# sxyu/pixel-nerf

Hardware: NVIDIA H100
Metric: rays/sec (64c+32f samples, 2 src views) (higher is better)
Workload: dtype f32 (fp16 hi/lo split products, fp32 accumulate)

## Files before the change

### pixel-nerf_b200/csrc/pnr_field_tc.cu

```cuda
#include <cuda_fp16.h>
#include <stdlib.h>

#include "pnr_common.cuh"
#include "pnr_geom.cuh"
#include "pnr_ray_ops.cuh"
#include "pnr_tc_ptx.cuh"

namespace pnr {

int sgemm(const float* A, int lda, const float* W, const float* bias, float* C, int ldc, int M, int N, int K,
          bool relu_a, bool accum, cudaStream_t s);
int gemm_f16x3(const float* A, int lda, const float* W, int ldw, const float* bias, float* C, int ldc, int M, int N, int K,
               cudaStream_t s);

namespace tc {

constexpr int D = 512;
constexpr int ROWS = 64;
constexpr int TILE_POINTS = 128;
constexpr int NCONSUMER_WARPS = 8;
constexpr int NCONSUMERS = NCONSUMER_WARPS * 32;
constexpr int NTHREADS = NCONSUMERS;
constexpr int SLOT_BYTES = 16384;
constexpr int HALF_SLOT_BYTES = SLOT_BYTES / 2;
constexpr int NSLOTS = 4;
constexpr int A_CHUNK_BYTES = 16384;
constexpr int A_BYTES = 8 * A_CHUNK_BYTES;
constexpr int AH_BYTES = 2 * A_CHUNK_BYTES;
constexpr int SLOTS_LIN_IN = 8;
constexpr int SLOTS_BLOCK = 128;
constexpr int SLOTS_TOTAL = SLOTS_LIN_IN + 5 * SLOTS_BLOCK;
constexpr int SLOTS_HEAD = SLOTS_LIN_IN + 3 * SLOTS_BLOCK;
constexpr int SLOTS_TAIL = 2 * SLOTS_BLOCK;
constexpr int HEADER_BYTES = 256;

constexpr int SM_A = 0;
constexpr int SM_AH = SM_A + A_BYTES;
constexpr int SM_B = SM_AH + AH_BYTES;
constexpr int SM_GEO = SM_B + NSLOTS * SLOT_BYTES;
constexpr int SM_PART = SM_A;
constexpr int SM_BAR = SM_GEO + ROWS * 8 * 4;
constexpr int BAR_FULL = 0;
constexpr int BAR_COUNT = BAR_FULL + NSLOTS;
constexpr int SM_NLIST = SM_BAR + 2 * BAR_COUNT * 8;
constexpr int SM_FEED = SM_NLIST + 16;
constexpr int FEED_BYTES = 128;
constexpr int SM_PROF = SM_FEED + 2 * FEED_BYTES;
#ifdef PNR_TC_PROFILE
constexpr int SMEM_BYTES = SM_PROF + 128;
#else
constexpr int SMEM_BYTES = SM_PROF;
#endif
static_assert(SMEM_BYTES <= 227 * 1024, "shared memory of one H100 block");
constexpr int FLUSH_SCRATCH_BYTES = A_BYTES / NCONSUMER_WARPS;


struct Pass {
  const uint8_t* packed;
  const float* proj;
  const float* fc0_b[5];
  const float* fc1_b[5];
  const float* lin_out_w;
  const float* lin_out_b;
  float* out;
  int64_t total_points;
  int64_t n_tiles;
  int64_t P;
  int K;
};

struct Render {
  const float* rays;
  const float *lin, *u_c, *u_f, *u_j, *n_d;
  float *zc, *wc, *zf;
  float *rgb_c, *depth_c, *rgb_f, *depth_f, *w_f;
  int* count;
  int* ready;
  int* lists;
  int64_t R;
  int cap, Kc, Kf, Kfd, white;
  float depth_std;
};

struct Params {
  PnrScene sc;
  PointSource src;
  Pass pass[2];
  Render rn;
  float* scratch;
  int npass;
  int* status;
};

using namespace tcptx;

enum { MODE_GATHER = 0, MODE_BIAS_WB = 1, MODE_COMBINE = 2, MODE_OUT = 3 };

#ifdef PNR_TC_PROFILE
extern __shared__ __align__(1024) uint8_t smem[];
enum { PH_FULL, PH_REFILL, PH_WGMMA_WAIT, PH_SYNC, PH_GATHER, PH_GEOM, PH_FLUSH, PH_TOTAL, PH_COUNT };
__device__ __forceinline__ void prof_add(int ph, long long t0, bool any_thread = false) {
  const long long dt = clock64() - t0;
  if (any_thread || (threadIdx.x & 127) == 0)
    reinterpret_cast<unsigned long long*>(smem + SM_PROF)[(threadIdx.x >> 7) * PH_COUNT + ph] += (unsigned long long)dt;
}
__device__ __forceinline__ void prof_finish(int* status, long long t_kernel) {
  prof_add(PH_TOTAL, t_kernel);
  if ((threadIdx.x & 127) == 0) {
    const unsigned long long* c = reinterpret_cast<const unsigned long long*>(smem + SM_PROF) + (threadIdx.x >> 7) * PH_COUNT;
    for (int i = 0; i < PH_COUNT; ++i) atomicAdd(reinterpret_cast<unsigned long long*>(status + 2) + i, c[i]);
  }
}
#define PROF_BEGIN(t) long long t = clock64()
#define PROF_RESTART(t) t = clock64()
#define PROF_END(ph, t) prof_add(ph, t)
#define PROF_END_ANY(ph, t) prof_add(ph, t, true)
#define PROF_INIT() \
  if (threadIdx.x < 2 * PH_COUNT) reinterpret_cast<unsigned long long*>(smem + SM_PROF)[threadIdx.x] = 0
#define PROF_FINISH(status, t) prof_finish(status, t)
#else
#define PROF_BEGIN(t)
#define PROF_RESTART(t)
#define PROF_END(ph, t)
#define PROF_END_ANY(ph, t)
#define PROF_INIT()
#define PROF_FINISH(status, t)
#endif

__device__ __forceinline__ void workers_sync() {
  PROF_BEGIN(t0);
  asm volatile("bar.sync 1, 256;" ::: "memory");
  PROF_END(PH_SYNC, t0);
}

__device__ __forceinline__ void st_evict_last(float* q, float v, uint64_t pol) {
  asm volatile("st.global.L2::cache_hint.f32 [%0], %1, %2;" ::"l"(q), "f"(v), "l"(pol) : "memory");
}
__device__ __forceinline__ float ld_evict_last(const float* q, uint64_t pol) {
  float v;
  asm volatile("ld.global.L2::cache_hint.f32 %0, [%1], %2;" : "=f"(v) : "l"(q), "l"(pol) : "memory");
  return v;
}
__device__ __forceinline__ float4 ldg_stream4(const float4* q, uint64_t pol) {
  float4 v;
  asm volatile("ld.global.nc.L2::cache_hint.v4.f32 {%0, %1, %2, %3}, [%4], %5;"
               : "=f"(v.x), "=f"(v.y), "=f"(v.z), "=f"(v.w)
               : "l"(q), "l"(pol));
  return v;
}
__device__ __forceinline__ void st_shared_u32(uint32_t saddr, uint32_t v) {
  asm volatile("st.shared.b32 [%0], %1;" ::"r"(saddr), "r"(v) : "memory");
}
__device__ __forceinline__ void split_relu2(float y0, float y1, uint32_t& hi, uint32_t& lo) {
  const float a0 = fmaxf(y0, 0.f), a1 = fmaxf(y1, 0.f);
  asm("cvt.rn.satfinite.f16x2.f32 %0, %1, %2;" : "=r"(hi) : "f"(a1), "f"(a0));
  const float2 hf = __half22float2(*reinterpret_cast<const __half2*>(&hi));
  asm("cvt.rn.satfinite.f16x2.f32 %0, %1, %2;" : "=r"(lo) : "f"(a1 - hf.y), "f"(a0 - hf.x));
}
__device__ __forceinline__ uint32_t relu_f16x2(float y0, float y1) {
  uint32_t hi;
  asm("cvt.rn.satfinite.f16x2.f32 %0, %1, %2;" : "=r"(hi) : "f"(fmaxf(y1, 0.f)), "f"(fmaxf(y0, 0.f)));
  return hi;
}
__device__ __forceinline__ uint32_t swz(int m, int k) {
  return (uint32_t)(m * 128 + ((((k >> 3) ^ (m & 7))) << 4) + (k & 7) * 2);
}

extern __shared__ __align__(1024) uint8_t smem[];

struct Feed {
  const uint8_t* src;
  uint64_t keep;
  int left;
  uint32_t released[2];
  const uint8_t* slots[2];
  int64_t n_tiles[2];
  int64_t tile;
  int npass, NS, pair, n_pairs;
  int ps, v;
  __device__ __forceinline__ void begin_run() {
    while (ps < npass && tile >= n_tiles[ps]) {
      ++ps;
      tile = pair;
    }
    const bool head = v < NS;
    src = ps < npass ? slots[ps] + (head ? 0 : (size_t)SLOTS_HEAD * SLOT_BYTES) : nullptr;
    left = (head ? SLOTS_HEAD : SLOTS_TAIL) / 2;
  }
  __device__ __forceinline__ void next_run() {
    if (++v > NS) {
      v = 0;
      tile += n_pairs;
    }
    begin_run();
  }
};
static_assert(sizeof(Feed) <= FEED_BYTES, "Feed does not fit its shared-memory slot");
static_assert(SLOTS_HEAD % 2 == 0 && SLOTS_TAIL % 2 == 0, "a step's two slots lie in one run");
static_assert(SM_PROF <= SMEM_BYTES, "the two rings' barriers and cursors fit under the block limit");
__device__ __forceinline__ Feed& feed(int wg) { return *reinterpret_cast<Feed*>(smem + SM_FEED + wg * FEED_BYTES); }

__device__ __forceinline__ uint32_t atom_add_acq_rel(uint32_t saddr, uint32_t v) {
  uint32_t old;
  asm volatile("atom.acq_rel.cta.shared::cta.add.u32 %0, [%1], %2;" : "=r"(old) : "r"(saddr), "r"(v) : "memory");
  return old;
}

template <bool FAST>
__device__ __forceinline__ void refill(uint32_t bar_base, uint32_t b_base, uint32_t n, int wg) {
  Feed& f = feed(wg);
  const uint8_t* src = f.src;
  if (src == nullptr) return;
  const uint64_t keep = f.keep;
  const uint32_t sl = n % NSLOTS;
#pragma unroll
  for (uint32_t k = 0; k < (FAST ? 1u : 2u); ++k) {
    const uint32_t full = bar_base + (BAR_FULL + sl + k) * 8;
    mbar_expect_tx(full, HALF_SLOT_BYTES);
    bulk_g2s_hint(b_base + (sl + k) * SLOT_BYTES, src + k * SLOT_BYTES, HALF_SLOT_BYTES, full, keep);
  }
  const int left = f.left - 1;
  f.left = left;
  if (left == 0)
    f.next_run();
  else
    f.src = src + 2 * SLOT_BYTES;
}

template <bool FAST>
struct Ring {
  uint32_t bar_base, b_base;
  uint32_t seq;
  uint32_t pend;
  bool has_pend;
  int lane;
  int* status;
  __device__ __forceinline__ uint32_t slot_addr(uint32_t s) const { return b_base + (s % NSLOTS) * SLOT_BYTES; }
  __device__ __forceinline__ void acquire() {
    if (has_pend) {
      PROF_BEGIN(t1);
      wgmma_wait<0>();
      PROF_END(PH_WGMMA_WAIT, t1);
      release(pend);
      has_pend = false;
    }
    PROF_BEGIN(t0);
    for (uint32_t s = seq; s < seq + (FAST ? 1 : 2); ++s)
      mbar_wait(bar_base + (BAR_FULL + s % NSLOTS) * 8, (s / NSLOTS) & 1, status,
                210 + 4 * (int)(threadIdx.x >> 7) + (int)(s % NSLOTS));
    PROF_END(PH_FULL, t0);
  }
  __device__ __forceinline__ void release(uint32_t s) {
    __syncwarp();
    if (lane == 0) {
      const int wg = threadIdx.x >> 7;
      if (atom_add_acq_rel(smem_u32(&feed(wg).released[(s / 2) & 1]), 1) % 4 == 3) {
        PROF_BEGIN(t0);
        refill<FAST>(bar_base, b_base, s + NSLOTS, wg);
        PROF_END_ANY(PH_REFILL, t0);
      }
    }
    __syncwarp();
  }
  __device__ __forceinline__ void issued() {
    wgmma_commit();
    pend = seq;
    has_pend = true;
    seq += 2;
  }
  __device__ __forceinline__ void drain() {
    PROF_BEGIN(t0);
    wgmma_wait<0>();
    PROF_END(PH_WGMMA_WAIT, t0);
    if (has_pend) release(pend);
    has_pend = false;
  }
};

template <bool FAST, int KSTEPS>
__device__ __forceinline__ void mma3(float* acc, uint64_t a_hi, uint64_t b_hi, uint64_t b_lo, bool zero) {
  const uint64_t a_lo = a_hi + (8192 >> 4);
#pragma unroll
  for (int kk = 0; kk < KSTEPS; ++kk) {
    wgmma_m64n64_f16(acc, a_hi + 2 * kk, b_hi + 2 * kk, (zero && kk == 0) ? 0u : 1u);
    if (FAST) continue;
    wgmma_m64n64_f16(acc, a_lo + 2 * kk, b_hi + 2 * kk, 1u);
    wgmma_m64n64_f16(acc, a_hi + 2 * kk, b_lo + 2 * kk, 1u);
  }
}

struct Cons {
  uint32_t smem_u;
  int tid, wg, lane;
  int r0, c0;
  float w_scale, w_inv;
  uint64_t l2_keep;
};

template <typename T>
__device__ __forceinline__ T* opaque(T* v) {
  asm volatile("" : "+l"(v));
  return v;
}
__device__ __forceinline__ uint32_t opaque(uint32_t v) {
  asm volatile("" : "+r"(v));
  return v;
}
__device__ __forceinline__ uint32_t acc_base(const Cons& c, uint32_t buf) {
  return opaque(c.smem_u + buf + c.wg * A_CHUNK_BYTES + swz(c.r0, c.c0));
}
__device__ __forceinline__ uint32_t acc_addr(uint32_t base, int q, int i) {
  return (base ^ (uint32_t)((i >> 2) << 4)) + q * 2 * A_CHUNK_BYTES + ((i >> 1) & 1) * 1024;
}

template <bool FAST, int KSTEPS>
__device__ __forceinline__ void wide_steps(Ring<FAST>& rg, const Cons& c, float (&x)[4][32], uint64_t a_hi,
                                           bool zero) {
  const uint64_t desc0 = make_desc(0);
#pragma unroll
  for (int q = 0; q < 4; ++q) {
    rg.acquire();
    const uint64_t b_hi = desc0 + (rg.slot_addr(rg.seq) >> 4);
    const uint64_t b_lo = desc0 + (rg.slot_addr(rg.seq + 1) >> 4);
    fence_acc<32>(x[q]);
    wgmma_fence();
    mma3<FAST, KSTEPS>(x[q], a_hi, b_hi, b_lo, zero);
    rg.issued();
  }
}

template <bool FAST>
__device__ __forceinline__ void fc_block(Ring<FAST>& rg, const Cons& c, float (&x)[4][32],
                                         const float* __restrict__ b0, const int* status) {
  const uint64_t desc0 = make_desc(0);
  float h[32];
#pragma unroll 1
  for (int hc = 0; hc < 4; ++hc) {
#pragma unroll 1
    for (int j = 0; j < 8; ++j) {
      rg.acquire();
      const uint64_t a_hi = desc0 + ((c.smem_u + SM_A + j * A_CHUNK_BYTES) >> 4);
      const uint64_t b_hi = desc0 + (rg.slot_addr(rg.seq) >> 4);
      const uint64_t b_lo = desc0 + (rg.slot_addr(rg.seq + 1) >> 4);
      fence_acc<32>(h);
      wgmma_fence();
      mma3<FAST, 4>(h, a_hi, b_hi, b_lo, j == 0);
      rg.issued();
    }
    rg.drain();
    fence_acc<32>(h);
    workers_sync();
    const float* bc = opaque(b0 + hc * 128 + c.wg * 64 + c.c0);
    const uint32_t ah = acc_base(c, SM_AH);
#pragma unroll
    for (int i = 0; i < 32; i += 2) {
      const float2 bb = __ldg(reinterpret_cast<const float2*>(bc + 8 * (i >> 2)));
      if (FAST) {
        st_shared_u32(acc_addr(ah, 0, i), relu_f16x2(h[i] * c.w_inv + bb.x, h[i + 1] * c.w_inv + bb.y));
        continue;
      }
      uint32_t hi, lo;
      split_relu2(h[i] * c.w_inv + bb.x, h[i + 1] * c.w_inv + bb.y, hi, lo);
      const uint32_t a = acc_addr(ah, 0, i);
      st_shared_u32(a, hi);
      st_shared_u32(a + 8192, lo);
    }
    fence_proxy_async();
    workers_sync();
#pragma unroll 1
    for (int jj = 0; jj < 2; ++jj)
      wide_steps<FAST, 4>(rg, c, x, desc0 + ((c.smem_u + SM_AH + jj * A_CHUNK_BYTES) >> 4), false);
  }
}

__device__ __forceinline__ void stage_gather(uint32_t smem_u, const float* __restrict__ proj_i, int warp, int lane) {
  const int sub = lane >> 4, l16 = lane & 15;
  uint64_t stream;
  asm volatile("createpolicy.fractional.L2::evict_first.b64 %0, 1.0;" : "=l"(stream));
#pragma unroll 1
  for (int j = 0; j < 8; ++j) {
    float4 t[4][4];
    uint32_t geo[4][4];
    float w[4][4];
#pragma unroll
    for (int it = 0; it < 4; ++it) {
      const uint32_t ga = smem_u + SM_GEO + (warp * 8 + it * 2 + sub) * 32;
#pragma unroll
      for (int k = 0; k < 4; ++k) {
        uint32_t wb;
        asm volatile("ld.shared.b32 %0, [%1];" : "=r"(geo[it][k]) : "r"(ga + 4 * k));
        asm volatile("ld.shared.b32 %0, [%1];" : "=r"(wb) : "r"(ga + 16 + 4 * k));
        w[it][k] = __uint_as_float(wb);
      }
    }
#pragma unroll
    for (int it = 0; it < 4; ++it)
#pragma unroll
      for (int k = 0; k < 4; ++k)
        t[it][k] = ldg_stream4(reinterpret_cast<const float4*>(proj_i + geo[it][k] + j * 64) + l16, stream);
#pragma unroll
    for (int it = 0; it < 4; ++it) {
      const int row = warp * 8 + it * 2 + sub;
      float4 g;
      g.x = ((t[it][0].x * w[it][0] + t[it][1].x * w[it][1]) + t[it][2].x * w[it][2]) + t[it][3].x * w[it][3];
      g.y = ((t[it][0].y * w[it][0] + t[it][1].y * w[it][1]) + t[it][2].y * w[it][2]) + t[it][3].y * w[it][3];
      g.z = ((t[it][0].z * w[it][0] + t[it][1].z * w[it][1]) + t[it][2].z * w[it][2]) + t[it][3].z * w[it][3];
      g.w = ((t[it][0].w * w[it][0] + t[it][1].w * w[it][1]) + t[it][2].w * w[it][2]) + t[it][3].w * w[it][3];
      const uint32_t a = smem_u + SM_A + j * A_CHUNK_BYTES + swz(row, (l16 >> 1) * 8) + ((l16 & 1) ? 8192u : 0u);
      asm volatile("st.shared.v4.f32 [%0], {%1, %2, %3, %4};" ::"r"(a), "f"(g.x), "f"(g.y), "f"(g.z), "f"(g.w) : "memory");
    }
  }
}

template <bool FAST, int MODE>
__device__ __forceinline__ void epilogue_x(Ring<FAST>& rg, const Cons& c, float (&x)[4][32], const float* __restrict__ bias,
                                           const float* __restrict__ proj_i, const float* __restrict__ lin_out_w,
                                           int view, int NS, float* __restrict__ scratch, float* out_part) {
  rg.drain();
#pragma unroll
  for (int q = 0; q < 4; ++q) fence_acc<32>(x[q]);
  workers_sync();
  const bool produce = (MODE != MODE_OUT) && !(MODE == MODE_COMBINE && view != NS - 1);
  if (MODE == MODE_GATHER) {
    PROF_BEGIN(t0);
    stage_gather(c.smem_u, proj_i, c.tid >> 5, c.lane);
    PROF_END(PH_GATHER, t0);
    workers_sync();
  }
  float o[2][4] = {{0.f, 0.f, 0.f, 0.f}, {0.f, 0.f, 0.f, 0.f}};
  const uint32_t xa = acc_base(c, SM_A);
  const uint32_t ga = opaque(c.smem_u + SM_A + c.wg * A_CHUNK_BYTES + swz(c.r0, 0) + (c.c0 >= 4 ? 8192u : 0u) +
                             (c.c0 & 3) * 4);
  const float* bp = MODE == MODE_GATHER ? nullptr : opaque(bias + 64 * c.wg + c.c0);
  const float* wp = MODE == MODE_OUT ? opaque(lin_out_w + 64 * c.wg + c.c0) : nullptr;
  float* sp0 = MODE == MODE_COMBINE ? opaque(scratch + c.tid) : nullptr;
#pragma unroll
  for (int q = 0; q < 4; ++q) {
#pragma unroll
    for (int i = 0; i < 32; i += 2) {
      const int r = (i >> 1) & 1;
      float y0 = x[q][i] * c.w_inv, y1 = x[q][i + 1] * c.w_inv;
      if (MODE == MODE_GATHER) {
        float2 g;
        asm volatile("ld.shared.v2.f32 {%0, %1}, [%2];" : "=f"(g.x), "=f"(g.y) : "r"(acc_addr(ga, q, i)) : "memory");
        __syncwarp();
        y0 += g.x;
        y1 += g.y;
      } else {
        const float2 bb = __ldg(reinterpret_cast<const float2*>(bp + 128 * q + 8 * (i >> 2)));
        y0 += bb.x;
        y1 += bb.y;
      }
      if (MODE == MODE_COMBINE && NS > 1) {
        float* sp = sp0 + (q * 32 + i) * NCONSUMERS;
        if (view == 0) {
          st_evict_last(sp, y0, c.l2_keep);
          st_evict_last(sp + NCONSUMERS, y1, c.l2_keep);
        } else {
          y0 = ld_evict_last(sp, c.l2_keep) + y0;
          y1 = ld_evict_last(sp + NCONSUMERS, c.l2_keep) + y1;
          if (view < NS - 1) {
            st_evict_last(sp, y0, c.l2_keep);
            st_evict_last(sp + NCONSUMERS, y1, c.l2_keep);
          } else {
            const float ns = (float)NS;
            y0 = y0 / ns;
            y1 = y1 / ns;
          }
        }
      }
      if (MODE == MODE_OUT) {
        const float a0 = fmaxf(y0, 0.f), a1 = fmaxf(y1, 0.f);
#pragma unroll
        for (int k = 0; k < 4; ++k) {
          const float2 w = __ldg(reinterpret_cast<const float2*>(wp + k * D + 128 * q + 8 * (i >> 2)));
          o[r][k] = fmaf(a1, w.y, fmaf(a0, w.x, o[r][k]));
        }
      } else if (produce) {
        x[q][i] = y0 * c.w_scale;
        x[q][i + 1] = y1 * c.w_scale;
        if (FAST) {
          st_shared_u32(acc_addr(xa, q, i), relu_f16x2(y0, y1));
          continue;
        }
        uint32_t hi, lo;
        split_relu2(y0, y1, hi, lo);
        const uint32_t a = acc_addr(xa, q, i);
        st_shared_u32(a, hi);
        st_shared_u32(a + 8192, lo);
      }
    }
  }
  if (MODE == MODE_OUT) {
#pragma unroll
    for (int r = 0; r < 2; ++r)
#pragma unroll
      for (int k = 0; k < 4; ++k) {
        o[r][k] += __shfl_xor_sync(0xffffffffu, o[r][k], 1);
        o[r][k] += __shfl_xor_sync(0xffffffffu, o[r][k], 2);
      }
    if ((c.lane & 3) == 0) {
#pragma unroll
      for (int r = 0; r < 2; ++r)
        reinterpret_cast<float4*>(out_part)[(c.r0 + 8 * r) * 2 + c.wg] = make_float4(o[r][0], o[r][1], o[r][2], o[r][3]);
    }
  } else if (produce) {
    fence_proxy_async();
  }
  workers_sync();
}

struct LdCg {
  __device__ __forceinline__ float operator()(const float* q) const { return __ldcg(q); }
};
struct LdCg4 {
  __device__ __forceinline__ float4 operator()(const float4* q) const { return __ldcg(q); }
};

__device__ __forceinline__ void finish_ray(const Params& p, int ps, int64_t ray, float* scratch, int lane) {
  const Render& rn = p.rn;
  const float* rr = rn.rays + ray * 8;
  const float near = rr[6], far = rr[7];
  const int Kc = rn.Kc, K = rn.Kc + rn.Kf;
  const int Kp = ps == 0 ? Kc : K;
  const float* zg = ps == 0 ? rn.zc + ray * Kc : rn.zf + ray * K;
  const float4* fg = reinterpret_cast<const float4*>(p.pass[ps].out) + ray * Kp;
  float* wg = ps == 0 ? rn.wc + ray * Kc : (rn.w_f ? rn.w_f + ray * K : nullptr);
  float* rgb = ps == 0 ? rn.rgb_c + ray * 3 : rn.rgb_f + ray * 3;
  float* dep = ps == 0 ? rn.depth_c + ray : rn.depth_f + ray;
  const bool staged = (size_t)(6 * Kp + Kc + 1 + K) * sizeof(float) <= (size_t)FLUSH_SCRATCH_BYTES;
  float4* fs = reinterpret_cast<float4*>(scratch);
  float* zs = scratch + 4 * Kp;
  float* ws = zs + Kp;
  float* rs = staged ? ws + Kp : scratch;
  if (staged) {
    for (int k = lane; k < Kp; k += 32) {
      fs[k] = __ldcg(fg + k);
      zs[k] = __ldcg(zg + k);
    }
    __syncwarp();
    if (lane == 0) composite_ray(zs, fs, far, Kp, rn.white, ws, rgb, dep, LdPlain(), LdPlain4());
    __syncwarp();
    if (wg)
      for (int k = lane; k < Kp; k += 32) wg[k] = ws[k];
  } else {
    if (lane == 0) composite_ray(zg, fg, far, Kp, rn.white, wg, rgb, dep, LdCg(), LdCg4());
    __syncwarp();
  }
  if (ps == 0 && p.npass > 1) {
    const int Ku = rn.Kf - rn.Kfd;
    const float dc = rn.Kfd > 0 ? __ldcg(rn.depth_c + ray) : 0.f;
    if (staged)
      sample_fine_ray(near, far, zs, ws, dc, rn.u_f + ray * Ku, rn.u_j + ray * Ku, rn.n_d + ray * rn.Kfd, rn.depth_std,
                      rn.zf + ray * K, Kc, rn.Kf, rn.Kfd, rs, lane, LdPlain());
    else
      sample_fine_ray(near, far, zg, wg, dc, rn.u_f + ray * Ku, rn.u_j + ray * Ku, rn.n_d + ray * rn.Kfd, rn.depth_std,
                      rn.zf + ray * K, Kc, rn.Kf, rn.Kfd, rs, lane, LdCg());
    __threadfence();
    __syncwarp();
    if (lane == 0) *reinterpret_cast<volatile int*>(rn.ready + ray) = 1;
  }
}

template <bool FAST>
__device__ __forceinline__ void field_tc(const Params& p) {
  const int warp = threadIdx.x >> 5, lane = threadIdx.x & 31;
  const int rank = blockIdx.x & 1;
  const int pair = blockIdx.x >> 1;
  const int n_pairs = gridDim.x >> 1;
  const int wg = threadIdx.x >> 7;
  const uint32_t bar_base = smem_u32(smem + SM_BAR) + wg * BAR_COUNT * 8;
  const uint32_t b_base = smem_u32(smem + SM_B) + wg * HALF_SLOT_BYTES;
  int* n_list = reinterpret_cast<int*>(smem + SM_NLIST);
  const int NS = p.sc.NS;
  const bool render = p.rn.rays != nullptr;
  PROF_BEGIN(t_kernel);
  PROF_INIT();

  if ((threadIdx.x & 127) == 0) {
    for (int i = 0; i < NSLOTS; ++i) mbar_init(bar_base + (BAR_FULL + i) * 8, 1);
    if (threadIdx.x == 0) *n_list = 0;
    Feed& f = feed(wg);
    for (int i = 0; i < 2; ++i) {
      f.slots[i] = i < p.npass ? p.pass[i].packed + HEADER_BYTES + wg * HALF_SLOT_BYTES : nullptr;
      f.n_tiles[i] = i < p.npass ? p.pass[i].n_tiles : 0;
    }
    asm volatile("createpolicy.fractional.L2::evict_last.b64 %0, 1.0;" : "=l"(f.keep));
    f.released[0] = f.released[1] = 0;
    f.npass = p.npass;
    f.NS = NS;
    f.pair = pair;
    f.n_pairs = n_pairs;
    f.ps = 0;
    f.v = 0;
    f.tile = pair;
    f.begin_run();
    asm volatile("fence.mbarrier_init.release.cluster;" ::: "memory");
  }
  __syncthreads();
  if ((threadIdx.x & 127) == 0) {
    refill<FAST>(bar_base, b_base, 0, wg);
    refill<FAST>(bar_base, b_base, 2, wg);
  }
  const size_t map_stride = (size_t)p.sc.SB * NS * p.sc.Hl * p.sc.Wl * D;

  {
    Cons c;
    c.smem_u = smem_u32(smem);
    c.tid = threadIdx.x;
    c.wg = threadIdx.x >> 7;
    c.lane = lane;
    c.r0 = 16 * (warp & 3) + (lane >> 2);
    c.c0 = 2 * (lane & 3);
    asm volatile("createpolicy.fractional.L2::evict_last.b64 %0, 1.0;" : "=l"(c.l2_keep));
    Ring<FAST> rg;
    rg.bar_base = bar_base;
    rg.b_base = b_base;
    rg.seq = 0;
    rg.pend = 0;
    rg.has_pend = false;
    rg.lane = lane;
    rg.status = p.status;
    float x[4][32];
    float* scratch = p.scratch + (size_t)blockIdx.x * D * ROWS;
    float* out_part = reinterpret_cast<float*>(smem + SM_PART);
    const int grow = threadIdx.x & 63;
    const int gsub = threadIdx.x >> 6;
    const uint64_t a0_desc = make_desc(c.smem_u + SM_A);

    for (int ps = 0; ps < p.npass; ++ps) {
      const Pass& P = p.pass[ps];
      c.w_scale = reinterpret_cast<const float*>(P.packed)[0];
      c.w_inv = reinterpret_cast<const float*>(P.packed)[1];
      for (int64_t tile = pair; tile < P.n_tiles; tile += n_pairs) {
        PROF_BEGIN(t_geo);
        const int64_t pt_raw = tile * TILE_POINTS + rank * ROWS + grow;
        const int64_t pt = pt_raw < P.total_points ? pt_raw : P.total_points - 1;
        const int sb = (int)(pt / P.P);
        float xp[3], d[3];
        if (render) {
          const int64_t ray = pt / P.K;
          const int k = (int)(pt - ray * P.K);
          const float* rr = p.rn.rays + ray * 8;
          float zz;
          if (ps == 0) {
            zz = coarse_sample(rr[6], rr[7], p.rn.lin ? p.rn.lin[k] : lin_step_value(k, P.K), p.rn.u_c[pt], P.K);
            if (gsub == 0 && pt_raw < P.total_points) p.rn.zc[pt] = zz;
          } else {
            if (gsub == 0 && (k == 0 || grow == 0) && pt_raw < P.total_points) {
              const volatile int* flag = p.rn.ready + ray;
              if (*flag == 0) {
                const long long t0 = clock64();
                uint32_t spins = 0;
                while (*flag == 0) {
                  __nanosleep(400);
                  if ((++spins & 0xFF) == 0) {
                    if (*(volatile int*)p.status != 0) break;
                    if (clock64() - t0 > timeout_limit(p.status)) {
                      atomicCAS(p.status, 0, 160);
                      if (((volatile int*)p.status)[1]) __trap();
                      break;
                    }
                  }
                }
              }
              __threadfence();
            }
            PROF_END(PH_GEOM, t_geo);
            workers_sync();
            PROF_RESTART(t_geo);
            zz = __ldcg(p.rn.zf + pt);
          }
          for (int i = 0; i < 3; ++i) {
            d[i] = rr[3 + i];
            xp[i] = __fadd_rn(rr[i], __fmul_rn(zz, d[i]));
          }
        } else {
          load_point(p.src, pt, xp, d);
        }
        PROF_END(PH_GEOM, t_geo);
        for (int v = 0; v < NS; ++v) {
          workers_sync();
          {
            PROF_BEGIN(t0);
            PointGeom pg = point_geometry(p.sc, sb, v, xp, d);
            if (gsub == 0) {
              uint32_t* geo = reinterpret_cast<uint32_t*>(smem + SM_GEO) + grow * 8;
              const uint32_t vbase = (uint32_t)(sb * NS + v) * p.sc.Hl * p.sc.Wl;
              geo[0] = (vbase + pg.y0 * p.sc.Wl + pg.x0) * D;
              geo[1] = (vbase + pg.y0 * p.sc.Wl + pg.x1) * D;
              geo[2] = (vbase + pg.y1 * p.sc.Wl + pg.x0) * D;
              geo[3] = (vbase + pg.y1 * p.sc.Wl + pg.x1) * D;
              geo[4] = __float_as_uint(pg.w_nw);
              geo[5] = __float_as_uint(pg.w_ne);
              geo[6] = __float_as_uint(pg.w_sw);
              geo[7] = __float_as_uint(pg.w_se);
            }
            uint8_t* row_hi = smem + SM_A + grow * 128;
            uint8_t* row_lo = row_hi + 8192;
#pragma unroll 1
            for (int e = 0; e < 12; e += 2) {
              const int ch = gsub * 12 + e;
              float f0 = feat_channel(pg, ch), f1 = feat_channel(pg, ch + 1);
              f0 = fmaxf(fminf(f0, 65504.f), -65504.f);
              f1 = fmaxf(fminf(f1, 65504.f), -65504.f);
              __half h0 = __float2half_rn(f0), h1 = __float2half_rn(f1);
              __half l0 = __float2half_rn(f0 - __half2float(h0)), l1 = __float2half_rn(f1 - __half2float(h1));
              const uint32_t hi = (uint32_t)__half_as_ushort(h0) | ((uint32_t)__half_as_ushort(h1) << 16);
              const uint32_t lo = (uint32_t)__half_as_ushort(l0) | ((uint32_t)__half_as_ushort(l1) << 16);
              const uint32_t byte = swz(grow, ch);
              *reinterpret_cast<uint32_t*>(row_hi - grow * 128 + byte) = hi;
              if (!FAST) *reinterpret_cast<uint32_t*>(row_lo - grow * 128 + byte) = lo;
            }
            fence_proxy_async();
            PROF_END(PH_GEOM, t0);
            workers_sync();
          }
#pragma unroll
          for (int q = 0; q < 4; ++q)
#pragma unroll
            for (int i = 0; i < 32; ++i) x[q][i] = 0.f;
          wide_steps<FAST, 3>(rg, c, x, a0_desc, true);
          epilogue_x<FAST, MODE_GATHER>(rg, c, x, nullptr, P.proj, nullptr, v, NS, nullptr, nullptr);
          for (int blk = 0; blk < 3; ++blk) {
            fc_block(rg, c, x, P.fc0_b[blk], p.status);
            if (blk < 2)
              epilogue_x<FAST, MODE_GATHER>(rg, c, x, nullptr, P.proj + (size_t)(blk + 1) * map_stride, nullptr, v,
                                            NS, nullptr, nullptr);
            else
              epilogue_x<FAST, MODE_COMBINE>(rg, c, x, P.fc1_b[2], nullptr, nullptr, v, NS, scratch, nullptr);
          }
        }
        fc_block(rg, c, x, P.fc0_b[3], p.status);
        epilogue_x<FAST, MODE_BIAS_WB>(rg, c, x, P.fc1_b[3], nullptr, nullptr, 0, NS, nullptr, nullptr);
        fc_block(rg, c, x, P.fc0_b[4], p.status);
        epilogue_x<FAST, MODE_OUT>(rg, c, x, P.fc1_b[4], nullptr, P.lin_out_w, 0, NS, nullptr, out_part);
        if (threadIdx.x < ROWS) {
          const int64_t opt = tile * TILE_POINTS + rank * ROWS + threadIdx.x;
          if (opt < P.total_points) {
            const float4 a = reinterpret_cast<const float4*>(out_part)[threadIdx.x * 2];
            const float4 b = reinterpret_cast<const float4*>(out_part)[threadIdx.x * 2 + 1];
            const float* bo = P.lin_out_b;
            const float r0 = (a.x + b.x) + bo[0], r1 = (a.y + b.y) + bo[1], r2 = (a.z + b.z) + bo[2],
                        r3 = (a.w + b.w) + bo[3];
            float4 o;
            o.x = 1.0f / (1.0f + expf(-r0));
            o.y = 1.0f / (1.0f + expf(-r1));
            o.z = 1.0f / (1.0f + expf(-r2));
            o.w = fmaxf(r3, 0.f);
            reinterpret_cast<float4*>(P.out)[opt] = o;
            if (render) __threadfence();
          }
        }
        workers_sync();
        if (render && threadIdx.x < ROWS) {
          const int64_t opt = tile * TILE_POINTS + rank * ROWS + threadIdx.x;
          if (opt < P.total_points) {
            const int64_t ray = opt / P.K;
            const int k = (int)(opt - ray * P.K);
            if (k == 0 || threadIdx.x == 0) {
              int64_t seg = P.K - k;
              if (seg > ROWS - (int)threadIdx.x) seg = ROWS - (int)threadIdx.x;
              if (seg > P.total_points - opt) seg = P.total_points - opt;
              const int old = atomicAdd(p.rn.count + (size_t)ps * p.rn.R + ray, (int)seg);
              if (old + (int)seg == P.K) {
                const int idx = atomicAdd(n_list, 1);
                p.rn.lists[(size_t)blockIdx.x * p.rn.cap + idx] = (int)ray;
              }
            }
          }
        }
      }
      if (render) {
        workers_sync();
        const int n_done = *reinterpret_cast<volatile int*>(n_list);
        __threadfence();
        float* fs = reinterpret_cast<float*>(smem + SM_A + warp * FLUSH_SCRATCH_BYTES);
        PROF_BEGIN(t0);
        for (int i = warp; i < n_done; i += NCONSUMER_WARPS)
          finish_ray(p, ps, p.rn.lists[(size_t)blockIdx.x * p.rn.cap + i], fs, lane);
        PROF_END(PH_FLUSH, t0);
        workers_sync();
        if (threadIdx.x == 0) *n_list = 0;
      }
    }
  }
  PROF_FINISH(p.status, t_kernel);
}

__global__ void __launch_bounds__(NTHREADS, 1) k_field_tc(const __grid_constant__ Params p) { field_tc<false>(p); }
__global__ void __launch_bounds__(NTHREADS, 1) k_field_tc_fast(const __grid_constant__ Params p) { field_tc<true>(p); }

__global__ void k_absmax(const float* __restrict__ w, int n, unsigned int* out) {
  float m = 0.f;
  for (int i = blockIdx.x * blockDim.x + threadIdx.x; i < n; i += gridDim.x * blockDim.x) m = fmaxf(m, fabsf(w[i]));
  for (int o = 16; o > 0; o >>= 1) m = fmaxf(m, __shfl_xor_sync(0xffffffffu, m, o));
  if ((threadIdx.x & 31) == 0) atomicMax(out, __float_as_uint(m));
}

__global__ void k_pack_header(const unsigned int* absmax_bits, float* header) {
  float m = __uint_as_float(*absmax_bits);
  float s = 1.0f;
  if (m > 0.f && isfinite(m)) {
    int e = (int)floorf(log2f(16384.0f / m));
    e = max(0, min(e, 12));
    s = exp2f((float)e);
  }
  header[0] = s;
  header[1] = 1.0f / s;
}

__global__ void k_pack_slots(const float* __restrict__ W0, const float* __restrict__ W1, int K, uint8_t* __restrict__ dst,
                             const float* __restrict__ header) {
  const int s = blockIdx.x;
  const float* W;
  int part, n0, k0;
  if (W1 == nullptr) {
    const int q = s >> 1;
    W = W0;
    part = s & 1;
    n0 = 128 * q;
    k0 = 0;
  } else {
    const int hc = s >> 5, r = s & 31;
    if (r < 16) {
      W = W0;
      part = r & 1;
      n0 = 128 * hc;
      k0 = 64 * (r >> 1);
    } else {
      const int r2 = r - 16, q = (r2 >> 1) & 3, jj = r2 >> 3;
      W = W1;
      part = r2 & 1;
      n0 = 128 * q;
      k0 = 64 * (2 * hc + jj);
    }
  }
  uint8_t* out = dst + (size_t)s * SLOT_BYTES;
  const float sc = header[0];
  for (int idx = threadIdx.x; idx < 128 * 64; idx += blockDim.x) {
    const int i = idx >> 6, kk = idx & 63;
    const int n = n0 + i, k = k0 + kk;
    float w = (k < K) ? W[(size_t)n * K + k] * sc : 0.f;
    __half hi = __float2half_rn(w);
    __half val = part ? __float2half_rn(w - __half2float(hi)) : hi;
    const int byte = i * 128 + (((kk >> 3) ^ (i & 7)) * 16) + (kk & 7) * 2;
    *reinterpret_cast<__half*>(out + byte) = val;
  }
}

__global__ void k_proj_bias(const float* a, const float* b, float* out, int n) {
  int i = blockIdx.x * blockDim.x + threadIdx.x;
  if (i < n) out[i] = a[i] + b[i];
}

static int* g_status[64] = {nullptr};

static int get_status_buffer(int** out) {
  int dev = 0;
  PNR_CUDA(cudaGetDevice(&dev));
  if (dev < 0 || dev >= 64) {
    set_error("device index out of range");
    return PNR_ERR_INVALID;
  }
  if (!g_status[dev]) {
    PNR_CUDA(cudaMalloc(&g_status[dev], 256));
    PNR_CUDA(cudaMemset(g_status[dev], 0, 256));
    const int init[2] = {0, getenv("PNR_TC_NO_TRAP") ? 0 : 1};
    PNR_CUDA(cudaMemcpy(g_status[dev], init, sizeof(init), cudaMemcpyHostToDevice));
    const int mult = getenv("PNR_TC_TIMEOUT_MULT") ? atoi(getenv("PNR_TC_TIMEOUT_MULT")) : 1;
    PNR_CUDA(cudaMemcpy(g_status[dev] + 20, &mult, sizeof(int), cudaMemcpyHostToDevice));
  }
  *out = g_status[dev];
  return PNR_OK;
}

}

int tc_status_buffer(int** out) { return tc::get_status_buffer(out); }

bool tc_supported(const PnrScene& sc, const PnrMlp& m) {
  const unsigned long long map_elems = (unsigned long long)sc.SB * sc.NS * sc.Hl * sc.Wl * tc::D;
  return m.d_hidden == tc::D && m.d_latent == tc::D && sc.C == tc::D && m.d_in == 42 && m.d_out == 4 &&
         m.n_blocks == 5 && m.combine_layer == 3 && sc.NS >= 1 && sc.NS <= 64 && map_elems < (1ull << 32);
}

static int tc_pairs(int64_t n_tiles) {
  int dev = 0, sms = 132;
  cudaGetDevice(&dev);
  cudaDeviceGetAttribute(&sms, cudaDevAttrMultiProcessorCount, dev);
  int64_t pairs = sms / 2;
  if (pairs > n_tiles) pairs = n_tiles;
  return (int)(pairs < 1 ? 1 : pairs);
}

static size_t tc_packed_bytes() { return (size_t)tc::HEADER_BYTES + (size_t)tc::SLOTS_TOTAL * tc::SLOT_BYTES; }

size_t tc_workspace_bytes(const PnrScene&, const PnrMlp&, int64_t total_points) {
  int64_t n_tiles = (total_points + tc::TILE_POINTS - 1) / tc::TILE_POINTS;
  return (size_t)tc_pairs(n_tiles) * 2 * tc::D * tc::ROWS * sizeof(float) + 1024;
}

static void fill_pass(tc::Pass& P, const PnrMlp& mlp, const float* proj, float* out, int64_t total_points, int64_t P_obj,
                      int K) {
  P.packed = static_cast<const uint8_t*>(mlp.packed);
  P.proj = proj;
  for (int i = 0; i < 5; ++i) {
    P.fc0_b[i] = mlp.fc0_b[i];
    P.fc1_b[i] = mlp.fc1_b[i];
  }
  P.lin_out_w = mlp.lin_out_w;
  P.lin_out_b = mlp.lin_out_b;
  P.out = out;
  P.total_points = total_points;
  P.n_tiles = (total_points + tc::TILE_POINTS - 1) / tc::TILE_POINTS;
  P.P = P_obj;
  P.K = K;
}

static int tc_launch(tc::Params& p, int pairs, bool fast, cudaStream_t s) {
  int rc = tc::get_status_buffer(&p.status);
  if (rc) return rc;
  static bool attr_set[2][64] = {{false}};
  int dev = 0;
// ... 236 lines not shown
```

### pixel-nerf_b200/csrc/pnr_tc_ptx.cuh

```cuda
#pragma once
#include <cuda_fp16.h>
#include <stdint.h>

namespace pnr {
namespace tcptx {

constexpr long long TIMEOUT_CYCLES = 4000000000LL;
__device__ __forceinline__ long long timeout_limit(const int* status) {
  const int m = ((const volatile int*)status)[20];
  return TIMEOUT_CYCLES * (long long)(m > 1 ? m : 1);
}

__device__ __forceinline__ uint32_t smem_u32(const void* p) { return (uint32_t)__cvta_generic_to_shared(p); }

__device__ __forceinline__ void mbar_init(uint32_t bar, uint32_t count) {
  asm volatile("mbarrier.init.shared::cta.b64 [%0], %1;" ::"r"(bar), "r"(count) : "memory");
}
__device__ __forceinline__ void mbar_arrive(uint32_t bar) {
  asm volatile("mbarrier.arrive.shared::cta.b64 _, [%0];" ::"r"(bar) : "memory");
}
__device__ __forceinline__ void mbar_expect_tx(uint32_t bar, uint32_t bytes) {
  asm volatile("mbarrier.arrive.expect_tx.shared::cta.b64 _, [%0], %1;" ::"r"(bar), "r"(bytes) : "memory");
}
__device__ __forceinline__ uint32_t mbar_try_wait(uint32_t bar, uint32_t parity) {
  uint32_t ok;
  asm volatile(
      "{\n\t.reg .pred p;\n\t"
      "mbarrier.try_wait.parity.shared::cta.b64 p, [%1], %2, %3;\n\t"
      "selp.u32 %0, 1, 0, p;\n\t}"
      : "=r"(ok)
      : "r"(bar), "r"(parity), "r"(0x989680u)
      : "memory");
  return ok;
}
static __device__ __noinline__ void mbar_wait_slow(uint32_t bar, uint32_t parity, int* status, int tag) {
  long long t0 = clock64();
  uint32_t spins = 0;
  while (!mbar_try_wait(bar, parity)) {
    if ((++spins & 0x3F) == 0) {
      if (*(volatile int*)status != 0) return;
      if (clock64() - t0 > timeout_limit(status)) {
        atomicCAS(status, 0, tag);
        if (((volatile int*)status)[1]) __trap();
        return;
      }
    }
  }
}
__device__ __forceinline__ void mbar_wait(uint32_t bar, uint32_t parity, int* status, int tag) {
  if (mbar_try_wait(bar, parity)) return;
  mbar_wait_slow(bar, parity, status, tag);
}

__device__ __forceinline__ void bulk_g2s(uint32_t dst, const void* src, uint32_t bytes, uint32_t bar) {
  asm volatile("cp.async.bulk.shared::cluster.global.mbarrier::complete_tx::bytes [%0], [%1], %2, [%3];" ::"r"(dst),
               "l"(src), "r"(bytes), "r"(bar)
               : "memory");
}
__device__ __forceinline__ void bulk_g2s_hint(uint32_t dst, const void* src, uint32_t bytes, uint32_t bar, uint64_t pol) {
  asm volatile(
      "cp.async.bulk.shared::cluster.global.mbarrier::complete_tx::bytes.L2::cache_hint [%0], [%1], %2, [%3], %4;" ::"r"(
          dst),
      "l"(src), "r"(bytes), "r"(bar), "l"(pol)
      : "memory");
}
__device__ __forceinline__ void fence_proxy_async() { asm volatile("fence.proxy.async.shared::cta;" ::: "memory"); }

__device__ __forceinline__ void wgmma_fence() { asm volatile("wgmma.fence.sync.aligned;" ::: "memory"); }
__device__ __forceinline__ void wgmma_commit() { asm volatile("wgmma.commit_group.sync.aligned;" ::: "memory"); }
template <int N>
__device__ __forceinline__ void wgmma_wait() {
  asm volatile("wgmma.wait_group.sync.aligned %0;" ::"n"(N) : "memory");
}
template <int N>
__device__ __forceinline__ void fence_acc(float* d) {
#pragma unroll
  for (int i = 0; i < N; ++i) asm volatile("" : "+f"(d[i])::"memory");
}

__device__ __forceinline__ uint64_t make_desc(uint32_t saddr) {
  uint64_t d = 0;
  d |= (uint64_t)((saddr >> 4) & 0x3FFF);
  d |= (uint64_t)1 << 16;
  d |= (uint64_t)(1024 >> 4) << 32;
  d |= (uint64_t)1 << 62;
  return d;
}

__device__ __forceinline__ void wgmma_m64n64_f16(float* d, uint64_t adesc, uint64_t bdesc, uint32_t accumulate) {
  asm volatile(
      "{\n\t.reg .pred p;\n\t"
      "setp.ne.b32 p, %34, 0;\n\t"
      "wgmma.mma_async.sync.aligned.m64n64k16.f32.f16.f16 "
      "{%0, %1, %2, %3, %4, %5, %6, %7, %8, %9, %10, %11, %12, %13, %14, %15, %16, %17, %18, %19, %20, %21, %22, %23, %24, %25, %26, %27, %28, %29, %30, %31}, "
      "%32, %33, p, 1, 1, 0, 0;\n\t}"
      : "+f"(d[0]), "+f"(d[1]), "+f"(d[2]), "+f"(d[3]), "+f"(d[4]), "+f"(d[5]), "+f"(d[6]), "+f"(d[7]), "+f"(d[8]), "+f"(d[9]), "+f"(d[10]), "+f"(d[11]), "+f"(d[12]), "+f"(d[13]), "+f"(d[14]), "+f"(d[15]), "+f"(d[16]), "+f"(d[17]), "+f"(d[18]), "+f"(d[19]), "+f"(d[20]), "+f"(d[21]), "+f"(d[22]), "+f"(d[23]), "+f"(d[24]), "+f"(d[25]), "+f"(d[26]), "+f"(d[27]), "+f"(d[28]), "+f"(d[29]), "+f"(d[30]), "+f"(d[31])
      : "l"(adesc), "l"(bdesc), "r"(accumulate));
}
__device__ __forceinline__ void wgmma_m64n128_f16(float* d, uint64_t adesc, uint64_t bdesc, uint32_t accumulate) {
  asm volatile(
      "{\n\t.reg .pred p;\n\t"
      "setp.ne.b32 p, %66, 0;\n\t"
      "wgmma.mma_async.sync.aligned.m64n128k16.f32.f16.f16 "
      "{%0, %1, %2, %3, %4, %5, %6, %7, %8, %9, %10, %11, %12, %13, %14, %15, %16, %17, %18, %19, %20, %21, %22, %23, %24, %25, %26, %27, %28, %29, %30, %31, %32, %33, %34, %35, %36, %37, %38, %39, %40, %41, %42, %43, %44, %45, %46, %47, %48, %49, %50, %51, %52, %53, %54, %55, %56, %57, %58, %59, %60, %61, %62, %63}, "
      "%64, %65, p, 1, 1, 0, 0;\n\t}"
      : "+f"(d[0]), "+f"(d[1]), "+f"(d[2]), "+f"(d[3]), "+f"(d[4]), "+f"(d[5]), "+f"(d[6]), "+f"(d[7]), "+f"(d[8]), "+f"(d[9]), "+f"(d[10]), "+f"(d[11]), "+f"(d[12]), "+f"(d[13]), "+f"(d[14]), "+f"(d[15]), "+f"(d[16]), "+f"(d[17]), "+f"(d[18]), "+f"(d[19]), "+f"(d[20]), "+f"(d[21]), "+f"(d[22]), "+f"(d[23]), "+f"(d[24]), "+f"(d[25]), "+f"(d[26]), "+f"(d[27]), "+f"(d[28]), "+f"(d[29]), "+f"(d[30]), "+f"(d[31]), "+f"(d[32]), "+f"(d[33]), "+f"(d[34]), "+f"(d[35]), "+f"(d[36]), "+f"(d[37]), "+f"(d[38]), "+f"(d[39]), "+f"(d[40]), "+f"(d[41]), "+f"(d[42]), "+f"(d[43]), "+f"(d[44]), "+f"(d[45]), "+f"(d[46]), "+f"(d[47]), "+f"(d[48]), "+f"(d[49]), "+f"(d[50]), "+f"(d[51]), "+f"(d[52]), "+f"(d[53]), "+f"(d[54]), "+f"(d[55]), "+f"(d[56]), "+f"(d[57]), "+f"(d[58]), "+f"(d[59]), "+f"(d[60]), "+f"(d[61]), "+f"(d[62]), "+f"(d[63])
      : "l"(adesc), "l"(bdesc), "r"(accumulate));
}
__device__ __forceinline__ void wgmma_m64n128_bf16(float* d, uint64_t adesc, uint64_t bdesc, uint32_t accumulate) {
  asm volatile(
      "{\n\t.reg .pred p;\n\t"
      "setp.ne.b32 p, %66, 0;\n\t"
      "wgmma.mma_async.sync.aligned.m64n128k16.f32.bf16.bf16 "
      "{%0, %1, %2, %3, %4, %5, %6, %7, %8, %9, %10, %11, %12, %13, %14, %15, %16, %17, %18, %19, %20, %21, %22, %23, %24, %25, %26, %27, %28, %29, %30, %31, %32, %33, %34, %35, %36, %37, %38, %39, %40, %41, %42, %43, %44, %45, %46, %47, %48, %49, %50, %51, %52, %53, %54, %55, %56, %57, %58, %59, %60, %61, %62, %63}, "
      "%64, %65, p, 1, 1, 0, 0;\n\t}"
      : "+f"(d[0]), "+f"(d[1]), "+f"(d[2]), "+f"(d[3]), "+f"(d[4]), "+f"(d[5]), "+f"(d[6]), "+f"(d[7]), "+f"(d[8]), "+f"(d[9]), "+f"(d[10]), "+f"(d[11]), "+f"(d[12]), "+f"(d[13]), "+f"(d[14]), "+f"(d[15]), "+f"(d[16]), "+f"(d[17]), "+f"(d[18]), "+f"(d[19]), "+f"(d[20]), "+f"(d[21]), "+f"(d[22]), "+f"(d[23]), "+f"(d[24]), "+f"(d[25]), "+f"(d[26]), "+f"(d[27]), "+f"(d[28]), "+f"(d[29]), "+f"(d[30]), "+f"(d[31]), "+f"(d[32]), "+f"(d[33]), "+f"(d[34]), "+f"(d[35]), "+f"(d[36]), "+f"(d[37]), "+f"(d[38]), "+f"(d[39]), "+f"(d[40]), "+f"(d[41]), "+f"(d[42]), "+f"(d[43]), "+f"(d[44]), "+f"(d[45]), "+f"(d[46]), "+f"(d[47]), "+f"(d[48]), "+f"(d[49]), "+f"(d[50]), "+f"(d[51]), "+f"(d[52]), "+f"(d[53]), "+f"(d[54]), "+f"(d[55]), "+f"(d[56]), "+f"(d[57]), "+f"(d[58]), "+f"(d[59]), "+f"(d[60]), "+f"(d[61]), "+f"(d[62]), "+f"(d[63])
      : "l"(adesc), "l"(bdesc), "r"(accumulate));
}

}
}
```

Measured before the change: 96480.

## Add dedicated producer warpgroup for weight TMA refills with register reallocation

Moves the bulk-copy refill of weight slots from the consumer warp that completes a release into a separate producer warpgroup. Two of its lanes each drive one ring, waiting on a shared-memory release counter before issuing the next copies. setmaxnreg lowers the producer's registers and raises the consumers' to 232, so the compute warps no longer stall on refill work and get more register room. The cost is an extra warpgroup per block and a spin-wait protocol on shared counters, which could add latency or hurt occupancy.

```diff
diff --git a/pixel-nerf_b200/csrc/pnr_field_tc.cu b/pixel-nerf_b200/csrc/pnr_field_tc.cu
--- a/pixel-nerf_b200/csrc/pnr_field_tc.cu
+++ b/pixel-nerf_b200/csrc/pnr_field_tc.cu
@@ -20,7 +20,11 @@
 constexpr int TILE_POINTS = 128;
 constexpr int NCONSUMER_WARPS = 8;
 constexpr int NCONSUMERS = NCONSUMER_WARPS * 32;
-constexpr int NTHREADS = NCONSUMERS;
+constexpr int NTHREADS = NCONSUMERS + 128;
+constexpr int PRODUCER_REGS = 40;
+constexpr int CONSUMER_REGS = 232;
+static_assert(128 * PRODUCER_REGS + NCONSUMERS * CONSUMER_REGS <= NTHREADS * 168,
+              "the consumers take no more registers than the producer returns");
 constexpr int SLOT_BYTES = 16384;
 constexpr int HALF_SLOT_BYTES = SLOT_BYTES / 2;
 constexpr int NSLOTS = 4;
@@ -42,10 +46,10 @@
 constexpr int SM_BAR = SM_GEO + ROWS * 8 * 4;
 constexpr int BAR_FULL = 0;
 constexpr int BAR_COUNT = BAR_FULL + NSLOTS;
-constexpr int SM_NLIST = SM_BAR + 2 * BAR_COUNT * 8;
-constexpr int SM_FEED = SM_NLIST + 16;
-constexpr int FEED_BYTES = 128;
-constexpr int SM_PROF = SM_FEED + 2 * FEED_BYTES;
+constexpr int RING_RELEASED = BAR_COUNT * 8;
+constexpr int RING_BYTES = RING_RELEASED + 8;
+constexpr int SM_NLIST = SM_BAR + 2 * RING_BYTES;
+constexpr int SM_PROF = SM_NLIST + 16;
 #ifdef PNR_TC_PROFILE
 constexpr int SMEM_BYTES = SM_PROF + 128;
 #else
@@ -99,9 +103,9 @@
 #ifdef PNR_TC_PROFILE
 extern __shared__ __align__(1024) uint8_t smem[];
 enum { PH_FULL, PH_REFILL, PH_WGMMA_WAIT, PH_SYNC, PH_GATHER, PH_GEOM, PH_FLUSH, PH_TOTAL, PH_COUNT };
-__device__ __forceinline__ void prof_add(int ph, long long t0, bool any_thread = false) {
+__device__ __forceinline__ void prof_add(int ph, long long t0) {
   const long long dt = clock64() - t0;
-  if (any_thread || (threadIdx.x & 127) == 0)
+  if ((threadIdx.x & 127) == 0)
     reinterpret_cast<unsigned long long*>(smem + SM_PROF)[(threadIdx.x >> 7) * PH_COUNT + ph] += (unsigned long long)dt;
 }
 __device__ __forceinline__ void prof_finish(int* status, long long t_kernel) {
@@ -114,17 +118,21 @@
 #define PROF_BEGIN(t) long long t = clock64()
 #define PROF_RESTART(t) t = clock64()
 #define PROF_END(ph, t) prof_add(ph, t)
-#define PROF_END_ANY(ph, t) prof_add(ph, t, true)
 #define PROF_INIT() \
   if (threadIdx.x < 2 * PH_COUNT) reinterpret_cast<unsigned long long*>(smem + SM_PROF)[threadIdx.x] = 0
 #define PROF_FINISH(status, t) prof_finish(status, t)
+#define PROF_SUM_INIT(s) long long s = 0
+#define PROF_SUM(s, t) s += clock64() - (t)
+#define PROF_PUBLISH(status, ph, s) atomicAdd(reinterpret_cast<unsigned long long*>((status) + 2) + (ph), (unsigned long long)(s))
 #else
 #define PROF_BEGIN(t)
 #define PROF_RESTART(t)
 #define PROF_END(ph, t)
-#define PROF_END_ANY(ph, t)
 #define PROF_INIT()
 #define PROF_FINISH(status, t)
+#define PROF_SUM_INIT(s)
+#define PROF_SUM(s, t)
+#define PROF_PUBLISH(status, ph, s)
 #endif
 
 __device__ __forceinline__ void workers_sync() {
@@ -170,35 +178,34 @@
 
 struct Feed {
   const uint8_t* src;
-  uint64_t keep;
+  int64_t tile;
   int left;
-  uint32_t released[2];
-  const uint8_t* slots[2];
-  int64_t n_tiles[2];
-  int64_t tile;
-  int npass, NS, pair, n_pairs;
   int ps, v;
-  __device__ __forceinline__ void begin_run() {
-    while (ps < npass && tile >= n_tiles[ps]) {
+  __device__ __forceinline__ void begin_run(const Params& p, int g) {
+    while (ps < p.npass && tile >= p.pass[ps].n_tiles) {
       ++ps;
-      tile = pair;
-    }
-    const bool head = v < NS;
-    src = ps < npass ? slots[ps] + (head ? 0 : (size_t)SLOTS_HEAD * SLOT_BYTES) : nullptr;
+      tile = blockIdx.x >> 1;
+    }
+    const bool head = v < p.sc.NS;
+    src = ps < p.npass ? p.pass[ps].packed + HEADER_BYTES + g * HALF_SLOT_BYTES +
+                             (head ? 0 : (size_t)SLOTS_HEAD * SLOT_BYTES)
+                       : nullptr;
     left = (head ? SLOTS_HEAD : SLOTS_TAIL) / 2;
   }
-  __device__ __forceinline__ void next_run() {
-    if (++v > NS) {
+  __device__ __forceinline__ void next(const Params& p, int g) {
+    if (--left > 0) {
+      src += 2 * SLOT_BYTES;
+      return;
+    }
+    if (++v > p.sc.NS) {
       v = 0;
-      tile += n_pairs;
-    }
-    begin_run();
+      tile += gridDim.x >> 1;
+    }
+    begin_run(p, g);
   }
 };
-static_assert(sizeof(Feed) <= FEED_BYTES, "Feed does not fit its shared-memory slot");
 static_assert(SLOTS_HEAD % 2 == 0 && SLOTS_TAIL % 2 == 0, "a step's two slots lie in one run");
-static_assert(SM_PROF <= SMEM_BYTES, "the two rings' barriers and cursors fit under the block limit");
-__device__ __forceinline__ Feed& feed(int wg) { return *reinterpret_cast<Feed*>(smem + SM_FEED + wg * FEED_BYTES); }
+static_assert(SM_PROF <= SMEM_BYTES, "the two rings' barriers and release counts fit under the block limit");
 
 __device__ __forceinline__ uint32_t atom_add_acq_rel(uint32_t saddr, uint32_t v) {
   uint32_t old;
@@ -207,33 +214,10 @@
 }
 
 template <bool FAST>
-__device__ __forceinline__ void refill(uint32_t bar_base, uint32_t b_base, uint32_t n, int wg) {
-  Feed& f = feed(wg);
-  const uint8_t* src = f.src;
-  if (src == nullptr) return;
-  const uint64_t keep = f.keep;
-  const uint32_t sl = n % NSLOTS;
-#pragma unroll
-  for (uint32_t k = 0; k < (FAST ? 1u : 2u); ++k) {
-    const uint32_t full = bar_base + (BAR_FULL + sl + k) * 8;
-    mbar_expect_tx(full, HALF_SLOT_BYTES);
-    bulk_g2s_hint(b_base + (sl + k) * SLOT_BYTES, src + k * SLOT_BYTES, HALF_SLOT_BYTES, full, keep);
-  }
-  const int left = f.left - 1;
-  f.left = left;
-  if (left == 0)
-    f.next_run();
-  else
-    f.src = src + 2 * SLOT_BYTES;
-}
-
-template <bool FAST>
 struct Ring {
   uint32_t bar_base, b_base;
   uint32_t seq;
-  uint32_t pend;
   bool has_pend;
-  int lane;
   int* status;
   __device__ __forceinline__ uint32_t slot_addr(uint32_t s) const { return b_base + (s % NSLOTS) * SLOT_BYTES; }
   __device__ __forceinline__ void acquire() {
@@ -241,7 +225,7 @@
       PROF_BEGIN(t1);
       wgmma_wait<0>();
       PROF_END(PH_WGMMA_WAIT, t1);
-      release(pend);
+      release(seq - 2);
       has_pend = false;
     }
     PROF_BEGIN(t0);
@@ -252,19 +236,11 @@
   }
   __device__ __forceinline__ void release(uint32_t s) {
     __syncwarp();
-    if (lane == 0) {
-      const int wg = threadIdx.x >> 7;
-      if (atom_add_acq_rel(smem_u32(&feed(wg).released[(s / 2) & 1]), 1) % 4 == 3) {
-        PROF_BEGIN(t0);
-        refill<FAST>(bar_base, b_base, s + NSLOTS, wg);
-        PROF_END_ANY(PH_REFILL, t0);
-      }
-    }
+    if ((threadIdx.x & 31) == 0) atom_add_acq_rel(bar_base + RING_RELEASED + ((s / 2) & 1) * 4, 1);
     __syncwarp();
   }
   __device__ __forceinline__ void issued() {
     wgmma_commit();
-    pend = seq;
     has_pend = true;
     seq += 2;
   }
@@ -272,10 +248,38 @@
     PROF_BEGIN(t0);
     wgmma_wait<0>();
     PROF_END(PH_WGMMA_WAIT, t0);
-    if (has_pend) release(pend);
+    if (has_pend) release(seq - 2);
     has_pend = false;
   }
 };
+
+template <bool FAST>
+__device__ __forceinline__ void produce(const Params& p, int g) {
+  const uint32_t bar_base = smem_u32(smem + SM_BAR) + g * RING_BYTES;
+  const uint32_t b_base = smem_u32(smem + SM_B) + g * HALF_SLOT_BYTES;
+  uint64_t keep;
+  asm volatile("createpolicy.fractional.L2::evict_last.b64 %0, 1.0;" : "=l"(keep));
+  Feed f;
+  f.tile = blockIdx.x >> 1;
+  f.ps = 0;
+  f.v = 0;
+  f.begin_run(p, g);
+  PROF_SUM_INIT(t_refill);
+  for (uint32_t s = 0; f.src != nullptr; ++s) {
+    const uint32_t pair = s & 1;
+    if (s >= 2) wait_count(bar_base + RING_RELEASED + pair * 4, 4 * (s >> 1), p.status, 220 + 2 * g + (int)pair);
+    PROF_BEGIN(t0);
+#pragma unroll
+    for (uint32_t k = 0; k < (FAST ? 1u : 2u); ++k) {
+      const uint32_t full = bar_base + (BAR_FULL + 2 * pair + k) * 8;
+      mbar_expect_tx(full, HALF_SLOT_BYTES);
+      bulk_g2s_hint(b_base + (2 * pair + k) * SLOT_BYTES, f.src + k * SLOT_BYTES, HALF_SLOT_BYTES, full, keep);
+    }
+    PROF_SUM(t_refill, t0);
+    f.next(p, g);
+  }
+  PROF_PUBLISH(p.status, PH_REFILL, t_refill);
+}
 
 template <bool FAST, int KSTEPS>
 __device__ __forceinline__ void mma3(float* acc, uint64_t a_hi, uint64_t b_hi, uint64_t b_lo, bool zero) {
@@ -569,7 +573,8 @@
   const int pair = blockIdx.x >> 1;
   const int n_pairs = gridDim.x >> 1;
   const int wg = threadIdx.x >> 7;
-  const uint32_t bar_base = smem_u32(smem + SM_BAR) + wg * BAR_COUNT * 8;
+  const bool producer = wg == 2;
+  const uint32_t bar_base = smem_u32(smem + SM_BAR) + wg * RING_BYTES;
   const uint32_t b_base = smem_u32(smem + SM_B) + wg * HALF_SLOT_BYTES;
   int* n_list = reinterpret_cast<int*>(smem + SM_NLIST);
   const int NS = p.sc.NS;
@@ -577,31 +582,20 @@
   PROF_BEGIN(t_kernel);
   PROF_INIT();
 
-  if ((threadIdx.x & 127) == 0) {
+  if (!producer && (threadIdx.x & 127) == 0) {
     for (int i = 0; i < NSLOTS; ++i) mbar_init(bar_base + (BAR_FULL + i) * 8, 1);
     if (threadIdx.x == 0) *n_list = 0;
-    Feed& f = feed(wg);
-    for (int i = 0; i < 2; ++i) {
-      f.slots[i] = i < p.npass ? p.pass[i].packed + HEADER_BYTES + wg * HALF_SLOT_BYTES : nullptr;
-      f.n_tiles[i] = i < p.npass ? p.pass[i].n_tiles : 0;
-    }
-    asm volatile("createpolicy.fractional.L2::evict_last.b64 %0, 1.0;" : "=l"(f.keep));
-    f.released[0] = f.released[1] = 0;
-    f.npass = p.npass;
-    f.NS = NS;
-    f.pair = pair;
-    f.n_pairs = n_pairs;
-    f.ps = 0;
-    f.v = 0;
-    f.tile = pair;
-    f.begin_run();
+    uint32_t* released = reinterpret_cast<uint32_t*>(smem + SM_BAR + wg * RING_BYTES + RING_RELEASED);
+    released[0] = released[1] = 0;
     asm volatile("fence.mbarrier_init.release.cluster;" ::: "memory");
   }
   __syncthreads();
-  if ((threadIdx.x & 127) == 0) {
-    refill<FAST>(bar_base, b_base, 0, wg);
-    refill<FAST>(bar_base, b_base, 2, wg);
-  }
+  if (producer) {
+    setmaxnreg_dec<PRODUCER_REGS>();
+    if (lane == 0 && warp < NCONSUMER_WARPS + 2) produce<FAST>(p, warp - NCONSUMER_WARPS);
+    return;
+  }
+  setmaxnreg_inc<CONSUMER_REGS>();
   const size_t map_stride = (size_t)p.sc.SB * NS * p.sc.Hl * p.sc.Wl * D;
 
   {
@@ -617,9 +611,7 @@
     rg.bar_base = bar_base;
     rg.b_base = b_base;
     rg.seq = 0;
-    rg.pend = 0;
     rg.has_pend = false;
-    rg.lane = lane;
     rg.status = p.status;
     float x[4][32];
     float* scratch = p.scratch + (size_t)blockIdx.x * D * ROWS;
diff --git a/pixel-nerf_b200/csrc/pnr_tc_ptx.cuh b/pixel-nerf_b200/csrc/pnr_tc_ptx.cuh
--- a/pixel-nerf_b200/csrc/pnr_tc_ptx.cuh
+++ b/pixel-nerf_b200/csrc/pnr_tc_ptx.cuh
@@ -6,9 +6,10 @@
 namespace tcptx {
 
 constexpr long long TIMEOUT_CYCLES = 4000000000LL;
-__device__ __forceinline__ long long timeout_limit(const int* status) {
+constexpr long long TIMEOUT_NS = 2000000000LL;
+__device__ __forceinline__ long long timeout_limit(const int* status, long long base = TIMEOUT_CYCLES) {
   const int m = ((const volatile int*)status)[20];
-  return TIMEOUT_CYCLES * (long long)(m > 1 ? m : 1);
+  return base * (long long)(m > 1 ? m : 1);
 }
 
 __device__ __forceinline__ uint32_t smem_u32(const void* p) { return (uint32_t)__cvta_generic_to_shared(p); }
@@ -33,6 +34,11 @@
       : "memory");
   return ok;
 }
+__device__ __forceinline__ uint32_t ld_acquire_shared(uint32_t saddr) {
+  uint32_t v;
+  asm volatile("ld.acquire.cta.shared::cta.u32 %0, [%1];" : "=r"(v) : "r"(saddr) : "memory");
+  return v;
+}
 static __device__ __noinline__ void mbar_wait_slow(uint32_t bar, uint32_t parity, int* status, int tag) {
   long long t0 = clock64();
   uint32_t spins = 0;
@@ -52,6 +58,31 @@
   mbar_wait_slow(bar, parity, status, tag);
 }
 
+__device__ __forceinline__ unsigned long long globaltimer_ns() {
+  unsigned long long t;
+  asm volatile("mov.u64 %0, %%globaltimer;" : "=l"(t));
+  return t;
+}
+static __device__ __noinline__ void wait_count_slow(uint32_t saddr, uint32_t target, int* status, int tag) {
+  const unsigned long long t0 = globaltimer_ns();
+  uint32_t spins = 0;
+  while (ld_acquire_shared(saddr) < target) {
+    __nanosleep(20);
+    if ((++spins & 0xFF) == 0) {
+      if (*(volatile int*)status != 0) return;
+      if (globaltimer_ns() - t0 > (unsigned long long)timeout_limit(status, TIMEOUT_NS)) {
+        atomicCAS(status, 0, tag);
+        if (((volatile int*)status)[1]) __trap();
+        return;
+      }
+    }
+  }
+}
+__device__ __forceinline__ void wait_count(uint32_t saddr, uint32_t target, int* status, int tag) {
+  if (ld_acquire_shared(saddr) >= target) return;
+  wait_count_slow(saddr, target, status, tag);
+}
+
 __device__ __forceinline__ void bulk_g2s(uint32_t dst, const void* src, uint32_t bytes, uint32_t bar) {
   asm volatile("cp.async.bulk.shared::cluster.global.mbarrier::complete_tx::bytes [%0], [%1], %2, [%3];" ::"r"(dst),
                "l"(src), "r"(bytes), "r"(bar)
@@ -65,6 +96,15 @@
       : "memory");
 }
 __device__ __forceinline__ void fence_proxy_async() { asm volatile("fence.proxy.async.shared::cta;" ::: "memory"); }
+
+template <uint32_t N>
+__device__ __forceinline__ void setmaxnreg_dec() {
+  asm volatile("setmaxnreg.dec.sync.aligned.u32 %0;" ::"n"(N));
+}
+template <uint32_t N>
+__device__ __forceinline__ void setmaxnreg_inc() {
+  asm volatile("setmaxnreg.inc.sync.aligned.u32 %0;" ::"n"(N));
+}
 
 __device__ __forceinline__ void wgmma_fence() { asm volatile("wgmma.fence.sync.aligned;" ::: "memory"); }
 __device__ __forceinline__ void wgmma_commit() { asm volatile("wgmma.commit_group.sync.aligned;" ::: "memory"); }
```

New measurement: 100,400 (median of 6 runs). 4.1% higher.
